# wongzbb/DiffMa-Diffusion-Mamba

Hardware: AMD Instinct MI355X
Metric: diffusion-steps/sec (DiffMa-L/2, 224x224, training; samples*steps/s) (higher is better)
Workload: dtype bf16 autocast (fp32 master weights, fp32 scan state); 1 GPU; DiffMa-L/2 DDP training step, 4x28x28 latents (196 tokens), batch 512/GPU; global_batch=512, seq_len=196, parallelism=dp1, gemm_tuning=file, world_size_seen_by_rccl=1

## Files before the change

### diffma-diffusion-mamba_amd/csrc/capi.hip

```cpp
#include "dm_common.h"
#include <cstdarg>
#include <cstdio>

namespace dm {
static thread_local char g_err[512] = "";
void set_error(const char* fmt, ...) {
    va_list ap;
    va_start(ap, fmt);
    vsnprintf(g_err, sizeof(g_err), fmt, ap);
    va_end(ap);
}
}

extern "C" int dm_abi_version(void) { return DM_ABI_VERSION; }
extern "C" const char* dm_last_error(void) { return dm::g_err; }
extern "C" const char* dm_build_info(void) {
#define DM_STR2(x) #x
#define DM_STR(x) DM_STR2(x)
    return "libdiffma_hip gfx950 (CDNA4, wave64) built " __DATE__ " " __TIME__ " hip " DM_STR(HIP_VERSION_MAJOR) "." DM_STR(
        HIP_VERSION_MINOR) "." DM_STR(HIP_VERSION_PATCH);
}
```

### diffma-diffusion-mamba_amd/csrc/conv_xproj.hip

```cpp
#include <cstdlib>
#include <type_traits>
#include "dm_mfma.h"

namespace dm {

constexpr int XP_TM = 16;
constexpr int XP_THREADS = 512;
constexpr int XP_PAD = 8;

template <typename T, typename TW, int W, bool SILU, int KSTEPS, bool IDX>
__global__ __launch_bounds__(XP_THREADS, 4) void conv_xproj_fwd_kernel(const dm_conv_xproj_fwd_args p) {
    constexpr int D = KSTEPS * 32;
    constexpr int KH = KSTEPS / 2;
    constexpr int ROW = D + XP_PAD;
    static_assert(KSTEPS % 2 == 0 && D <= 2 * XP_THREADS, "dim must be a multiple of 64 and at most 1024");
    __shared__ __attribute__((aligned(16))) uint16_t tile[2][XP_TM * ROW];
    __shared__ __attribute__((aligned(16))) f32x4 red[4][WAVE];

    const int tid = threadIdx.x;
    const int wave = __builtin_amdgcn_readfirstlane(tid >> 6), lane = tid & 63;
    const int nt = wave & 3, kh = wave >> 2;
    const int g = lane >> 4, ij = lane & 15;
    const int b = (int)blockIdx.x / p.ndir;
    const int dir = (int)blockIdx.x % p.ndir;
    const int s = dir * p.batch + b;
    const int L = p.seqlen;
    const cptr<int32_t> idx = IDX ? as_const(p.row_index + (int64_t)dir * L) : nullptr;
    const bool act = (D == 2 * XP_THREADS) ? true : (2 * tid < D);
    const int c = act ? 2 * tid : 0;
    const rsrc_t r_x = make_rsrc((const T*)p.x + (int64_t)b * p.x_sb);
    const rsrc_t r_o = make_rsrc((T*)p.out + (int64_t)s * p.o_ss);
    const int vo = c * (int)sizeof(T);
    const int sl_x = (int)p.x_sl * (int)sizeof(T), sl_o = (int)p.o_sl * (int)sizeof(T);
    const rsrc_t r_xd = make_rsrc((T*)p.xdbl + (int64_t)s * L * p.xd_sr);
    const int sr_xd = (int)p.xd_sr * (int)sizeof(T);

    const int ncol = p.nproj;
    const int col = nt * 16 + ij;
    const bool wave_on = nt * 16 < ncol;
    u32x4_t bfrag[KH];
    {
        const rsrc_t r_wx = __builtin_amdgcn_make_buffer_rsrc(const_cast<void*>(p.wx), 0, ncol * D * (int)sizeof(T), 0x00020000);
#pragma unroll
        for (int kk = 0; kk < KH; ++kk) {
            const auto q = __builtin_amdgcn_raw_buffer_load_b128(r_wx, (col * D + (kh * KH + kk) * 32 + g * 8) * (int)sizeof(T), 0, 0);
            bfrag[kk] = (u32x4_t){q[0], q[1], q[2], q[3]};
        }
    }

    float w[W][2], bias[2], win[W - 1][2];
#pragma unroll
    for (int v = 0; v < 2; ++v) {
#pragma unroll
        for (int j = 0; j < W; ++j) w[j][v] = io<TW>::ld((const TW*)p.weight + (int64_t)(c + v) * W + j);
        bias[v] = p.bias ? io<TW>::ld((const TW*)p.bias + c + v) : 0.0f;
#pragma unroll
        for (int j = 0; j < W - 1; ++j) win[j][v] = 0.0f;
    }

    auto load_half = [&](int l0, int h, uint32_t(&xin)[XP_TM]) {
#pragma unroll
        for (int j = h * (XP_TM / 2); j < (h + 1) * (XP_TM / 2); ++j) {
            int l = l0 + j;
            l = l < L ? l : L - 1;
            const int r = IDX ? idx[l] : l;
            xin[j] = __builtin_amdgcn_raw_buffer_load_b32(r_x, vo, r * sl_x, 0);
        }
    };
// ... 19 lines not shown
#pragma unroll
                for (int k = 0; k < W - 2; ++k) win[k][v] = win[k + 1][v];
                if (W > 1) win[W - 2][v] = xv[v];
            }
            const uint32_t pk = valid ? mfma<T>::pack(acc[0], acc[1]) : 0u;
            if (act) {
                *reinterpret_cast<uint32_t*>(tl + j * ROW + c) = pk;
                if (valid) __builtin_amdgcn_raw_buffer_store_b32(pk, r_o, vo, (l0 + j) * sl_o, 0);
            }
        }
        if (t + 1 < ntile) load_half(l0 + XP_TM, h, xin);
    };
    for (int t = 0; t < ntile; ++t) {
        const int l0 = t * XP_TM;
        uint16_t* const tl = tile[t & 1];
        conv_half(t, 0);
        conv_half(t, 1);
        __syncthreads();
        f32x4 acc = {0.f, 0.f, 0.f, 0.f};
        if (wave_on) {
#pragma unroll
            for (int kk = 0; kk < KH; ++kk) {
                const u32x4_t a = *reinterpret_cast<const u32x4_t*>(tl + ij * ROW + (kh * KH + kk) * 32 + g * 8);
                acc = mfma<T>::m16(a, bfrag[kk], acc);
            }
            if (kh == 1) red[nt][lane] = acc;
        }
        __syncthreads();
        if (wave_on && kh == 0 && col < ncol) {
            const f32x4 o = acc + red[nt][lane];
#pragma unroll
            for (int r = 0; r < 4; ++r) {
                const int l = l0 + 4 * g + r;
                if (l < L) bio<T>::st(r_xd, l * sr_xd + col * (int)sizeof(T), 0, o[r]);
            }
        }
    }
}

template <typename T, typename TW, int W, int KSTEPS>
static void launch_xp(const dm_conv_xproj_fwd_args& a, hipStream_t st) {
    dim3 grid(a.ndir * a.batch), block(XP_THREADS);
    const bool silu = (a.flags & DM_FLAG_SILU) != 0;
    if (a.row_index) {
        if (silu) hipLaunchKernelGGL((conv_xproj_fwd_kernel<T, TW, W, true, KSTEPS, true>), grid, block, 0, st, a);
        else hipLaunchKernelGGL((conv_xproj_fwd_kernel<T, TW, W, false, KSTEPS, true>), grid, block, 0, st, a);
    } else {
        if (silu) hipLaunchKernelGGL((conv_xproj_fwd_kernel<T, TW, W, true, KSTEPS, false>), grid, block, 0, st, a);
        else hipLaunchKernelGGL((conv_xproj_fwd_kernel<T, TW, W, false, KSTEPS, false>), grid, block, 0, st, a);
    }
}

template <typename T, typename TW, int W>
static int xp_by_dim(const dm_conv_xproj_fwd_args& a, hipStream_t st) {
    switch (a.dim) {
        case 1024: launch_xp<T, TW, W, 32>(a, st); break;
#ifndef DM_FAST_BUILD
        case 512: launch_xp<T, TW, W, 16>(a, st); break;
        case 256: launch_xp<T, TW, W, 8>(a, st); break;
#endif
        case 128: launch_xp<T, TW, W, 4>(a, st); break;
        default: set_error("dm_gather_conv1d_xproj_fwd: dim %d not instantiated (128, 256, 512, 1024)", a.dim); return DM_ERR_ARG;
    }
    return launch_status("dm_gather_conv1d_xproj_fwd");
}

template <typename T, typename TW>
// ... 8 lines not shown
    }
}

}

extern "C" int dm_gather_conv1d_xproj_width_supported(int width) {
#ifdef DM_FAST_BUILD
    return width == 4;
#else
    return width >= 2 && width <= 4;
#endif
}

extern "C" int dm_gather_conv1d_xproj_supported(int dim, int nproj, int io_dtype) {
    const bool d_ok = dim == 128 || dim == 256 || dim == 512 || dim == 1024;
    return (d_ok && nproj >= 1 && nproj <= 64 && (io_dtype == DM_BF16 || io_dtype == DM_F16)) ? 1 : 0;
}

extern "C" int dm_gather_conv1d_xproj_fwd(const dm_conv_xproj_fwd_args* args, void* stream) {
    using namespace dm;
    if (!args) { set_error("dm_gather_conv1d_xproj_fwd: null args"); return DM_ERR_ARG; }
    const dm_conv_xproj_fwd_args& a = *args;
    if (!a.x || !a.weight || !a.out || !a.wx || !a.xdbl) { set_error("dm_gather_conv1d_xproj_fwd: null tensor pointer"); return DM_ERR_ARG; }
    if (a.batch <= 0 || a.dim <= 0 || a.seqlen <= 0 || a.ndir <= 0) { set_error("dm_gather_conv1d_xproj_fwd: non-positive size"); return DM_ERR_ARG; }
    if (a.ndir > 1 && !a.row_index) { set_error("dm_gather_conv1d_xproj_fwd: ndir>1 needs row_index"); return DM_ERR_ARG; }
    if (!dm_gather_conv1d_xproj_supported(a.dim, a.nproj, a.io_dtype)) {
        set_error("dm_gather_conv1d_xproj_fwd: needs 16-bit I/O, dim in {128,256,512,1024}, nproj <= 64 (got dim %d nproj %d dtype %d)", a.dim, a.nproj, a.io_dtype);
        return DM_ERR_ARG;
    }
    if (a.x_sd != 1 || a.o_sd != 1) { set_error("dm_gather_conv1d_xproj_fwd: needs token-major tensors (channel stride 1)"); return DM_ERR_LAYOUT; }
    if (((uintptr_t)a.x & 3) || (a.x_sb & 1) || (a.x_sl & 1) || ((uintptr_t)a.out & 3) || (a.o_ss & 1) || (a.o_sl & 1) || ((uintptr_t)a.wx & 15)) {
        set_error("dm_gather_conv1d_xproj_fwd: x / out need 4-byte aligned rows, wx a 16-byte aligned base");
        return DM_ERR_LAYOUT;
    }
    hipStream_t st = (hipStream_t)stream;
    const bool wf32 = a.w_dtype == DM_F32;
    if (!wf32 && a.w_dtype != a.io_dtype) { set_error("dm_gather_conv1d_xproj_fwd: w_dtype must be fp32 or io_dtype"); return DM_ERR_DTYPE; }
    if (a.io_dtype == DM_BF16) return wf32 ? xp_by_width<bf16_t, float>(a, st) : xp_by_width<bf16_t, bf16_t>(a, st);
    return wf32 ? xp_by_width<f16_t, float>(a, st) : xp_by_width<f16_t, f16_t>(a, st);
}

namespace dm {

template <typename T, typename TW, int W, bool SILU, int D, bool IDX, bool MERGED = false>
__global__ __launch_bounds__(XP_THREADS, 2) void conv_xproj_bwd_kernel(const dm_conv_xproj_bwd_args p) {
    constexpr int NTW = D / 128;
    constexpr int ROWP = D + 4;
    constexpr int KP = 64;
    static_assert(D % 128 == 0 && D <= 2 * XP_THREADS, "dim must be a multiple of 128 and at most 1024");
    __shared__ __attribute__((aligned(16))) float ptile[XP_TM * ROWP];

    const int tid = threadIdx.x;
    const int wave = __builtin_amdgcn_readfirstlane(tid >> 6), lane = tid & 63;
    const int g = lane >> 4, ij = lane & 15;
    const int L = p.seqlen;
    const int b = MERGED ? (int)blockIdx.x : (int)blockIdx.x % p.batch;
    const bool act = (D == 2 * XP_THREADS) ? true : (2 * tid < D);
    const int c = act ? 2 * tid : 0;
    constexpr int ES = (int)sizeof(T);
    const rsrc_t r_x = make_rsrc((const T*)p.x + (int64_t)b * p.x_sb);
    const rsrc_t r_wt = make_rsrc(p.wxt);
    const int vo = c * ES;
    const int sl_x = (int)p.x_sl * ES, sl_du = (int)p.du_sl * ES, sl_dx = (int)p.dx_sl * ES, sr_xd = (int)p.xd_sr * ES;

    u32x4_t bfrag[NTW][2];
#pragma unroll
// ... 550 lines not shown
```

### diffma-diffusion-mamba_amd/csrc/dm_common.h

```cpp
#pragma once
#include <hip/hip_runtime.h>
#include <hip/hip_bf16.h>
#include <hip/hip_fp16.h>
#include <stdint.h>
#include "../../include/diffma_hip.h"

namespace dm {

constexpr int WAVE = 64;
constexpr float LOG2E = 1.4426950408889634f;
constexpr float LN2 = 0.6931471805599453f;

constexpr int DM_MAX_MIX = 2;
template <typename A> struct mix_args {
    A a[DM_MAX_MIX];
    int n;
};
void set_error(const char* fmt, ...);
static inline int launch_status(const char* who) {
    const hipError_t e = hipGetLastError();
    if (e == hipSuccess) return DM_OK;
    set_error("%s: launch failed: %s", who, hipGetErrorString(e));
    return DM_ERR_LAUNCH;
}
template <typename A> static inline mix_args<A> mix_make(const A& a, const A* second, unsigned& gz) {
    mix_args<A> m;
    m.a[0] = a;
    m.a[1] = second ? *second : a;
    m.n = second ? 2 : 1;
    gz = (unsigned)m.n;
    return m;
}
template <typename A, typename Check, typename Pairs, typename Run>
static inline int mix_run_n(const char* who, const A* args, int n, void* stream, Check check, Pairs pairs, Run run) {
    if (!args || n <= 0) { set_error("%s: null args / n <= 0", who); return DM_ERR_ARG; }
    for (int i = 0; i < n;) {
        int rc = check(args[i]);
        if (rc != 0) return rc;
        const bool pair = i + 1 < n && check(args[i + 1]) == 0 && pairs(args[i], args[i + 1]);
        rc = run(args[i], pair ? &args[i + 1] : nullptr, (hipStream_t)stream);
        if (rc != 0) return rc;
        i += pair ? 2 : 1;
    }
    return 0;
}
static inline bool same_align16(const void* x, const void* y) { return (((uintptr_t)x ^ (uintptr_t)y) & 15) == 0; }
static inline bool same_align4(const void* x, const void* y) { return (((uintptr_t)x ^ (uintptr_t)y) & 3) == 0; }
template <typename A, typename... M>
static inline bool mix_congruent(const A& x, const A& y, M A::*... ptrs) {
    if ((... || ((x.*ptrs == nullptr) != (y.*ptrs == nullptr)))) return false;
    A u = x, v = y;
    ((u.*ptrs = nullptr, v.*ptrs = nullptr), ...);
    return __builtin_memcmp(&u, &v, sizeof(A)) == 0;
}

typedef float f32x2 __attribute__((ext_vector_type(2)));
typedef float f32x4 __attribute__((ext_vector_type(4)));

struct bf16_t { uint16_t v; };
struct f16_t { _Float16 v; };

typedef __bf16 dm_bf16x2_t __attribute__((ext_vector_type(2)));
typedef float dm_f32x2_t __attribute__((ext_vector_type(2)));
__device__ __forceinline__ uint32_t dm_cvt_pk_bf16(float lo, float hi) {
    return __builtin_bit_cast(uint32_t, __builtin_convertvector((dm_f32x2_t){lo, hi}, dm_bf16x2_t));
}

__device__ __forceinline__ uint32_t f32_to_bf16_bits(float x) {
    return dm_cvt_pk_bf16(x, x) & 0xffffu;
}

template <typename T> struct io;
template <> struct io<float> {
    static __device__ __forceinline__ float ld(const float* p) { return *p; }
    static __device__ __forceinline__ void st(float* p, float x) { *p = x; }
    static __device__ __forceinline__ uint32_t ld_raw(const float* p) { return __float_as_uint(*p); }
    static __device__ __forceinline__ float cv(uint32_t w) { return __uint_as_float(w); }
};
template <> struct io<bf16_t> {
    static __device__ __forceinline__ float ld(const bf16_t* p) {
        return __uint_as_float(((uint32_t)p->v) << 16);
    }
    static __device__ __forceinline__ void st(bf16_t* p, float x) { p->v = (uint16_t)f32_to_bf16_bits(x); }
    static __device__ __forceinline__ uint32_t ld_raw(const bf16_t* p) { return (uint32_t)p->v; }
    static __device__ __forceinline__ float cv(uint32_t w) { return __uint_as_float(w << 16); }
};
template <> struct io<f16_t> {
    static __device__ __forceinline__ float ld(const f16_t* p) { return (float)p->v; }
    static __device__ __forceinline__ void st(f16_t* p, float x) { p->v = (_Float16)x; }
    static __device__ __forceinline__ uint32_t ld_raw(const f16_t* p) { return (uint32_t)__builtin_bit_cast(unsigned short, p->v); }
// ... 184 lines not shown
```

### diffma-diffusion-mamba_amd/csrc/scan_fwd_impl.h

```cpp
#pragma once
#include "dm_common.h"
#include <type_traits>

namespace dm {

#ifndef DM_FWD_F32_WAVES
#define DM_FWD_F32_WAVES 1
#endif

template <int N, bool HAS_Z, bool SOFTPLUS, bool ASH = false>
__device__ __forceinline__ float scan_step(f32x2 (&h)[N / 2], const f32x2 (&A2)[N / 2], const float (&Bv)[N],
                                           const float (&Cv)[N], float uu, float draw, float zz, float Dv, float bias) {
    float dl = draw + bias;
    if (SOFTPLUS) dl = softplus_f(dl);
    const float du = dl * uu;
    f32x2 acc = (f32x2){0.0f, 0.0f};
    float a_sh = 0.0f;
    if (ASH) a_sh = fast_exp2(A2[0].x * dl);
#pragma unroll
    for (int k = 0; k < N / 2; ++k) {
        f32x2 a;
        if (ASH) {
            a = (f32x2){a_sh, a_sh};
        } else {
            const f32x2 t = A2[k] * dl;
            a.x = fast_exp2(t.x);
            a.y = fast_exp2(t.y);
        }
        f32x2 bb, cc;
        bb.x = Bv[2 * k];
        bb.y = Bv[2 * k + 1];
        cc.x = Cv[2 * k];
        cc.y = Cv[2 * k + 1];
        h[k] = a * h[k] + bb * du;
        acc += h[k] * cc;
    }
    float y = acc.x + acc.y + Dv * uu;
    if (HAS_Z) y *= silu_f(zz);
    return y;
}

template <typename T, typename TBC, int N, bool HAS_Z, bool IDX, bool CKPT, bool SOFTPLUS, int PF, bool ASH = false, bool ACC = false>
__global__ __launch_bounds__(64) __attribute__((amdgpu_waves_per_eu((sizeof(T) == 2 && sizeof(TBC) == 2 && N <= 16) ? (ACC ? 3 : 4) : ((sizeof(T) == 4 && N <= 16) ? DM_FWD_F32_WAVES : 1)))) void scan_fwd_kernel(const dm_scan_fwd_args p) {
    static_assert(!ACC || IDX, "accumulating launches are built for the model's call pattern (row-index tables)");
    static_assert(N % 2 == 0, "d_state must be even");
    static_assert(PF == 8, "the B/C staging below maps 8 steps onto the 64 lanes");
    constexpr int NP = N / 2;
    constexpr int ES = (int)sizeof(T), EBC = (int)sizeof(TBC);
    constexpr int PER = N / 4;
    __shared__ __attribute__((aligned(16))) float bc_lds[2][PF][2 * N];
    const int d_raw = blockIdx.x * WAVE + threadIdx.x;
    const int d = (d_raw < p.dim) ? d_raw : p.dim - 1;
    const int L = p.seqlen;
    const int bpd = (p.batch_per_dir > 0) ? p.batch_per_dir : p.nseq;
    const int grp = (blockIdx.x * WAVE) / (p.dim / p.ngroups);
    const int s = blockIdx.y;
    const int dir = s / bpd;
    const int sb = s - dir * bpd;

    const rsrc_t r_u = make_rsrc((const T*)p.u + (int64_t)s * p.u_ss);
    const rsrc_t r_dt = make_rsrc((const T*)p.delta + (int64_t)s * p.dt_ss);
    const rsrc_t r_z = make_rsrc(HAS_Z ? (const T*)p.z + (int64_t)sb * p.z_ss : nullptr);
    const rsrc_t r_o = make_rsrc((T*)p.out + (int64_t)s * p.o_ss);
    const int vo = d * ES;
    const int sl_u = (int)p.u_sl * ES, sl_dt = (int)p.dt_sl * ES, sl_z = (int)p.z_sl * ES, sl_o = (int)p.o_sl * ES;
    const int lane = threadIdx.x;
    const int bc_step = lane >> 3, bc_part = lane & 7;
    const bool bc_isB = bc_part < 4;
    const rsrc_t r_bc = make_rsrc(bc_isB ? (const void*)((const TBC*)p.B + (int64_t)s * p.B_ss + (int64_t)grp * p.B_sg)
                                         : (const void*)((const TBC*)p.C + (int64_t)s * p.C_ss + (int64_t)grp * p.C_sg));
    const int sl_bc = (int)(bc_isB ? p.B_sl : p.C_sl) * EBC;
    const int vo_bc = (bc_part & 3) * PER * EBC;
    float* const bc_slot = &bc_lds[0][bc_step][(bc_isB ? 0 : N) + (bc_part & 3) * PER];
    const cptr<int32_t> zidx = IDX ? as_const(p.z_row_index + (int64_t)dir * L) : nullptr;
    const cptr<int32_t> oidx = IDX ? as_const(p.out_row_index + (int64_t)dir * L) : nullptr;

    f32x2 A2[NP];
#pragma unroll
    for (int j = 0; j < NP; ++j) {
        A2[j].x = p.A[(int64_t)d * N + 2 * j] * LOG2E;
        A2[j].y = p.A[(int64_t)d * N + 2 * j + 1] * LOG2E;
    }
    const float Dv = p.D ? p.D[d] : 0.0f;
    const float bias = p.delta_bias ? p.delta_bias[d] : 0.0f;

    f32x2 h[NP];
#pragma unroll
    for (int j = 0; j < NP; ++j) h[j] = (f32x2){0.0f, 0.0f};

    constexpr bool CK_PACKED = std::is_same<T, bf16_t>::value;
    constexpr int CK_ROWS = CK_PACKED ? NP : N;
    const int nchunk = CKPT ? (L + DM_SCAN_CKPT_EVERY - 1) / DM_SCAN_CKPT_EVERY : 0;
    const rsrc_t r_ck = make_rsrc(CKPT ? (const uint32_t*)p.ckpt + (int64_t)s * nchunk * CK_ROWS * p.dim : nullptr);
    auto store_slot = [&](int c) {
        if constexpr (CK_PACKED) {
            uint32_t w[NP];
#pragma unroll
            for (int k = 0; k < NP; ++k) asm("v_cvt_pk_bf16_f32 %0, %1, %2" : "=v"(w[k]) : "v"(h[k].x), "v"(h[k].y));
            bio_st_words<NP>(w, r_ck, d * 16, c * p.dim * NP * 4, p.dim * 16);
        } else {
#pragma unroll
            for (int k = 0; k < NP; ++k) {
                bio<float>::st(r_ck, d * 4, ((c * N + 2 * k) * p.dim) * 4, h[k].x);
                bio<float>::st(r_ck, d * 4, ((c * N + 2 * k + 1) * p.dim) * 4, h[k].y);
            }
        }
    };
    auto store_ckpt = [&](int done) {
        if (done < L) store_slot(done / DM_SCAN_CKPT_EVERY);
    };

    auto ld_old = [&](int l) -> float {
        if constexpr (ACC) return bio<T>::ld(r_o, vo, oidx[l] * sl_o);
        else return 0.0f;
    };
    float ru[PF], rd[PF], rz[PF], ro[ACC ? PF : 1];
#pragma unroll
    for (int j = 0; j < PF; ++j) {
        const int l = (j < L) ? j : L - 1;
        ru[j] = bio<T>::ld(r_u, vo, l * sl_u);
        rd[j] = bio<T>::ld(r_dt, vo, l * sl_dt);
        if (HAS_Z) rz[j] = bio<T>::ld(r_z, vo, (IDX ? zidx[l] : l) * sl_z);
        if (ACC) ro[j] = ld_old(l);
    }
    auto fetch_bc = [&](int l0, float(&v)[PER]) {
        int l = l0 + bc_step;
        l = (l < L) ? l : L - 1;
        bio_ld_vec<TBC, PER>(v, r_bc, vo_bc + l * sl_bc, 0);
    };
    auto stash_bc = [&](int b, const float(&v)[PER]) {
#pragma unroll
        for (int k = 0; k < PER; ++k) bc_slot[b * PF * 2 * N + k] = v[k];
    };
    {
        float v[PER];
        fetch_bc(0, v);
        stash_bc(0, v);
    }
    int buf = 0;

    auto run_block = [&](int l0, const float(&cu)[PF], const float(&cd)[PF], const float(&cz)[PF], const float(&co)[ACC ? PF : 1],
                         float(&nu)[PF], float(&nd)[PF], float(&nz)[PF], float(&no)[ACC ? PF : 1]) {
        float nbc[PER];
        fetch_bc(l0 + PF, nbc);
#pragma unroll
        for (int j = 0; j < PF; ++j) {
            int l = l0 + PF + j;
            l = (l < L) ? l : L - 1;
            nu[j] = bio<T>::ld(r_u, vo, l * sl_u);
            nd[j] = bio<T>::ld(r_dt, vo, l * sl_dt);
            if (HAS_Z) nz[j] = bio<T>::ld(r_z, vo, (IDX ? zidx[l] : l) * sl_z);
            if (ACC) no[j] = ld_old(l);
        }
#pragma unroll
        for (int j = 0; j < PF; ++j) {
            const int l = l0 + j;
            float Bc[N], Cc[N];
#pragma unroll
            for (int k = 0; k < N; ++k) {
                Bc[k] = bc_lds[buf][j][k];
                Cc[k] = bc_lds[buf][j][N + k];
            }
            float y = scan_step<N, HAS_Z, SOFTPLUS, ASH>(h, A2, Bc, Cc, cu[j], cd[j], HAS_Z ? cz[j] : 0.0f, Dv, bias);
            if (ACC) y += co[j];
            bio<T>::st(r_o, vo, (IDX ? oidx[l] : l) * sl_o, y);
            if (CKPT && (j + 1) % DM_SCAN_CKPT_EVERY == 0) store_ckpt(l0 + j + 1);
        }
        buf ^= 1;
        stash_bc(buf, nbc);
    };

    const int Lfull = (L / PF) * PF;
    float su[PF], sd[PF], sz[PF], so[ACC ? PF : 1];
    int l0 = 0;
    for (; l0 + 2 * PF <= Lfull; l0 += 2 * PF) {
        run_block(l0, ru, rd, rz, ro, su, sd, sz, so);
        run_block(l0 + PF, su, sd, sz, so, ru, rd, rz, ro);
    }
    if (l0 < Lfull) {
        run_block(l0, ru, rd, rz, ro, su, sd, sz, so);
#pragma unroll
        for (int j = 0; j < PF; ++j) {
            ru[j] = su[j];
            rd[j] = sd[j];
            if (HAS_Z) rz[j] = sz[j];
            if (ACC) ro[j] = so[j];
        }
    }
#pragma unroll
    for (int j = 0; j < PF; ++j) {
        const int l = Lfull + j;
        if (l < L) {
            float Bc[N], Cc[N];
#pragma unroll
            for (int k = 0; k < N; ++k) {
                Bc[k] = bc_lds[buf][j][k];
                Cc[k] = bc_lds[buf][j][N + k];
            }
            float y = scan_step<N, HAS_Z, SOFTPLUS, ASH>(h, A2, Bc, Cc, ru[j], rd[j], HAS_Z ? rz[j] : 0.0f, Dv, bias);
            if (ACC) y += ro[j];
            bio<T>::st(r_o, vo, (IDX ? oidx[l] : l) * sl_o, y);
            if (CKPT && (j + 1) % DM_SCAN_CKPT_EVERY == 0) store_ckpt(l + 1);
        }
    }

    if (CKPT) store_slot(0);

    if (p.last_state) {
        float* ls = p.last_state + ((int64_t)s * N) * p.dim + d;
#pragma unroll
        for (int k = 0; k < NP; ++k) {
            ls[(int64_t)(2 * k) * p.dim] = h[k].x;
            ls[(int64_t)(2 * k + 1) * p.dim] = h[k].y;
        }
    }
}

constexpr int SCAN_PF = 8;
static_assert(SCAN_PF % DM_SCAN_CKPT_EVERY == 0, "checkpoints fall on fixed positions of a prefetch block");

template <typename T, typename TBC, int N, bool HAS_Z, bool IDX>
static void launch_fwd3(const dm_scan_fwd_args& a, hipStream_t st, dim3 grid) {
    const bool sp = (a.flags & DM_FLAG_DELTA_SOFTPLUS) != 0;
    if constexpr (N == 16 && HAS_Z && IDX) {
        if ((a.flags & DM_FLAG_OUT_ACCUMULATE) && sp && !(a.flags & DM_FLAG_A_SHARED)) {
            if (a.ckpt) hipLaunchKernelGGL((scan_fwd_kernel<T, TBC, N, true, true, true, true, SCAN_PF, false, true>), grid, dim3(WAVE), 0, st, a);
            else hipLaunchKernelGGL((scan_fwd_kernel<T, TBC, N, true, true, false, true, SCAN_PF, false, true>), grid, dim3(WAVE), 0, st, a);
            return;
        }
    }
    if constexpr (N == 16 && HAS_Z && IDX) {
        if ((a.flags & DM_FLAG_A_SHARED) && sp) {
            if (a.ckpt) hipLaunchKernelGGL((scan_fwd_kernel<T, TBC, N, true, true, true, true, SCAN_PF, true>), grid, dim3(WAVE), 0, st, a);
            else hipLaunchKernelGGL((scan_fwd_kernel<T, TBC, N, true, true, false, true, SCAN_PF, true>), grid, dim3(WAVE), 0, st, a);
            return;
        }
    }
    if (a.ckpt) {
        if (sp) hipLaunchKernelGGL((scan_fwd_kernel<T, TBC, N, HAS_Z, IDX, true, true, SCAN_PF>), grid, dim3(WAVE), 0, st, a);
        else hipLaunchKernelGGL((scan_fwd_kernel<T, TBC, N, HAS_Z, IDX, true, false, SCAN_PF>), grid, dim3(WAVE), 0, st, a);
    } else {
        if (sp) hipLaunchKernelGGL((scan_fwd_kernel<T, TBC, N, HAS_Z, IDX, false, true, SCAN_PF>), grid, dim3(WAVE), 0, st, a);
        else hipLaunchKernelGGL((scan_fwd_kernel<T, TBC, N, HAS_Z, IDX, false, false, SCAN_PF>), grid, dim3(WAVE), 0, st, a);
    }
}

template <typename T, typename TBC, int N>
static int launch_fwd(const dm_scan_fwd_args& a, hipStream_t st) {
    dim3 grid((a.dim + WAVE - 1) / WAVE, a.nseq);
    const bool idx = a.z_row_index != nullptr;
    if (a.z) {
        if (idx) launch_fwd3<T, TBC, N, true, true>(a, st, grid);
        else launch_fwd3<T, TBC, N, true, false>(a, st, grid);
    } else {
        if (idx) launch_fwd3<T, TBC, N, false, true>(a, st, grid);
        else launch_fwd3<T, TBC, N, false, false>(a, st, grid);
    }
    return launch_status("dm_selective_scan_fwd");
}

template <typename T, typename TBC>
static int dispatch_n(const dm_scan_fwd_args& a, hipStream_t st) {
    switch (a.dstate) {
        case 16: return launch_fwd<T, TBC, 16>(a, st);
#ifndef DM_FAST_BUILD
        case 8: return launch_fwd<T, TBC, 8>(a, st);
        case 32: return launch_fwd<T, TBC, 32>(a, st);
        case 64: return launch_fwd<T, TBC, 64>(a, st);
#endif
        default:
            set_error("dm_selective_scan_fwd: d_state=%d not instantiated (8,16,32,64)", a.dstate);
            return DM_ERR_DSTATE;
    }
}

template <typename T>
static int dispatch_bc(const dm_scan_fwd_args& a, hipStream_t st) {
    if (a.bc_dtype == DM_F32) return dispatch_n<T, float>(a, st);
    if (a.bc_dtype == a.io_dtype) return dispatch_n<T, T>(a, st);
    set_error("dm_selective_scan_fwd: bc_dtype %d must be fp32 or equal io_dtype %d", a.bc_dtype, a.io_dtype);
    return DM_ERR_DTYPE;
}

// ... 2 lines not shown
```

### diffma-diffusion-mamba_amd/hip_ops.py

```python
from __future__ import annotations

import ctypes
import os
import threading

import torch

from . import _lib
from ._lib import (DM_BF16, DM_F16, DM_F32, DM_FLAG_A_SHARED, DM_FLAG_DELTA_ACTIVATED, DM_FLAG_DX_MERGED, DM_FLAG_PARTIAL_COMPACT, DM_FLAG_OUT_ACCUMULATE, DM_FLAG_DELTA_SOFTPLUS, DM_FLAG_DOUT_PER_SEQ, DM_FLAG_SCAN_CHUNKED, DM_FLAG_SCAN_SEQUENTIAL, DM_FLAG_SILU, dm_blend_args, dm_gate_head_args, dm_dtproj_bwd_args, dm_conv_bwd_args, dm_rmsnorm_merge_args, dm_colsum_args, dm_sum_partials_args,
                   dm_conv_fwd_args, dm_conv_xproj_bwd_args, dm_conv_xproj_fwd_args, dm_diffusion_step_args, dm_ln_mod_args, dm_ssd_bwd_args, dm_ssd_fwd_args, dm_merge_args, dm_gate_bwd_args, dm_dtproj_args, dm_scan_bwd_args, dm_scan_fwd_args, dm_gemm_args, dm_repack_args, dm_training_loss_args)

_DT = {torch.float32: DM_F32, torch.bfloat16: DM_BF16, torch.float16: DM_F16}
SCAN_CKPT_EVERY = _lib.DM_SCAN_CKPT_EVERY


def union_length(intervals):
    total, cur_s, cur_e = 0.0, None, None
    for s0, e0 in sorted(intervals):
        if cur_e is None or s0 > cur_e:
            if cur_e is not None:
                total += cur_e - cur_s
            cur_s, cur_e = s0, e0
        else:
            cur_e = max(cur_e, e0)
# ... 378 lines not shown
    Bsz, L, Dm = x.shape
    W = weight.shape[-1]
    weight = weight.reshape(Dm, W).contiguous()
    if weight.dtype != x.dtype and weight.dtype != torch.float32:
        weight = weight.float()
    if bias is not None:
        bias = bias.to(weight.dtype).contiguous()
    if out is None:
        out = torch.empty((ndir * Bsz, L, Dm), dtype=x.dtype, device=x.device)
    a = dm_conv_fwd_args()
    a.batch, a.dim, a.seqlen, a.width, a.ndir = Bsz, Dm, L, W, ndir
    a.io_dtype, a.w_dtype = dtype_code(x), dtype_code(weight)
    a.flags = DM_FLAG_SILU if silu else 0
    a.x, a.weight, a.bias, a.row_index, a.out = _ptr(x), _ptr(weight), _ptr(bias), _ptr(row_index), _ptr(out)
    a.x_sb, a.x_sl, a.x_sd = x.stride()
    a.o_ss, a.o_sl, a.o_sd = out.stride()
    _launch("dm_gather_conv1d_fwd", a, x, 2 * ndir * Bsz * L * Dm * x.element_size())
    return out


XPROJ_FUSED_MIN_SEQS = 512


def conv_xproj_supported(x, wx, nseq, width=4):
    if not x.is_cuda or x.dtype not in (torch.bfloat16, torch.float16) or nseq < XPROJ_FUSED_MIN_SEQS:
        return False
    if not _lib.load().dm_gather_conv1d_xproj_width_supported(int(width)):
        return False
    if x.stride(0) % 2 or x.stride(1) % 2 or x.storage_offset() % 2:
        return False
    return bool(_lib.load().dm_gather_conv1d_xproj_supported(int(x.shape[-1]), int(wx.shape[0]), dtype_code(x)))


def gather_conv1d_xproj_fwd(x, weight, bias, wx, *, row_index=None, ndir=1, silu=True):
    _require_gpu(x, weight, bias, wx)
    Bsz, L, Dm = x.shape
    W = weight.shape[-1]
    P = wx.shape[0]
    weight = weight.reshape(Dm, W).contiguous()
    if weight.dtype != x.dtype and weight.dtype != torch.float32:
        weight = weight.float()
    if bias is not None:
        bias = bias.to(weight.dtype).contiguous()
    wx = wx.contiguous()
    assert wx.dtype == x.dtype and wx.shape[1] == Dm
    out = torch.empty((ndir * Bsz, L, Dm), dtype=x.dtype, device=x.device)
    xdbl = torch.empty((ndir * Bsz * L, P), dtype=x.dtype, device=x.device)
    a = dm_conv_xproj_fwd_args()
    a.batch, a.dim, a.seqlen, a.width, a.ndir = Bsz, Dm, L, W, ndir
    a.io_dtype, a.w_dtype = dtype_code(x), dtype_code(weight)
    a.flags = DM_FLAG_SILU if silu else 0
    a.nproj = P
    a.x, a.weight, a.bias, a.row_index = _ptr(x), _ptr(weight), _ptr(bias), _ptr(row_index)
    a.wx, a.out, a.xdbl = _ptr(wx), _ptr(out), _ptr(xdbl)
    a.x_sb, a.x_sl, a.x_sd = x.stride()
    a.o_ss, a.o_sl, a.o_sd = out.stride()
    a.xd_sr = P
    es = x.element_size()
    _launch("dm_gather_conv1d_xproj_fwd", a, x, 2 * ndir * Bsz * L * Dm * es + ndir * Bsz * L * P * es + P * Dm * es)
    return out, xdbl


XPROJ_FUSED_BWD = os.environ.get("DIFFMA_FUSED_CONV_BWD", "1") == "1"


def conv_xproj_bwd_supported(x, wx, nseq, width=4, du=None, dxdbl=None):
    if not XPROJ_FUSED_BWD:
        return False
    if not _lib.load().dm_gather_conv1d_xproj_width_supported(int(width)):
        return False
    if du is not None and (du.data_ptr() % 4 or du.stride(0) % 2 or du.stride(1) % 2 or du.stride(2) != 1):
        return False
    if dxdbl is not None and (dxdbl.data_ptr() % 16 or dxdbl.stride(0) % 8 or dxdbl.stride(1) != 1):
        return False
    if not x.is_cuda or x.dtype not in (torch.bfloat16, torch.float16) or nseq < XPROJ_FUSED_MIN_SEQS:
        return False
    if x.stride(0) % 2 or x.stride(1) % 2 or x.storage_offset() % 2:
        return False
    return bool(_lib.load().dm_gather_conv1d_xproj_bwd_supported(int(x.shape[-1]), int(wx.shape[0]), dtype_code(x)))


DX_MERGED = os.environ.get("DIFFMA_DX_MERGED", "1") == "1"


def gather_conv1d_xproj_bwd(x, weight, bias, du, dxdbl, wxt, *, row_index=None, ndir=1, silu=True, merged_out=None):
    _require_gpu(x, weight, bias, du, dxdbl, wxt)
    Bsz, L, Dm = x.shape
    W = weight.shape[-1]
    P = wxt.shape[1]
    weight = weight.reshape(Dm, W).contiguous()
    if weight.dtype != x.dtype and weight.dtype != torch.float32:
        weight = weight.float()
    if bias is not None:
# ... 632 lines not shown
```

### diffma-diffusion-mamba_amd/selective_scan_interface.py

```python
from __future__ import annotations

import os

import torch
import torch.nn.functional as F

from . import _lib, hip_ops
from .step_prep import cast_weight, stacked_pair


REPACK_OWN = os.environ.get("DIFFMA_REPACK_OWN", "1") == "1"


def _repack_own(t: torch.Tensor) -> bool:
    return (REPACK_OWN and t.is_cuda and t.dim() == 3 and t.stride(2) == 1 and t.shape[0] <= 65535
            and t.dtype in (torch.float32, torch.bfloat16, torch.float16))


def _to_token_major(t: torch.Tensor) -> torch.Tensor:
    tm = t.transpose(1, 2)
    if tm.stride(-1) == 1:
        return tm
    if _repack_own(t):
        return hip_ops.repack(t, True)
# ... 232 lines not shown
                    dx = GemmChain.run(F.linear, dy2c, wt).view(xc.shape).to(x_dt)
            else:
                dx = GemmChain.run(torch.mm, dy2, wc).view(xc.shape).to(x_dt)
            if not ctx.needs_input_grad[1]:
                dw = None
            elif b_dt is None and _own_single(dy2c, x2c, False, False, torch.float32):
                dw = hip_ops.gemm(dy2c, x2c, False, False, out_dtype=torch.float32).to(w_dt)
            else:
                dw = _tn_splitk(dy2c, x2c).to(w_dt)
            db = dy2.sum(0, dtype=torch.float32).to(b_dt) if (b_dt is not None and ctx.needs_input_grad[2]) else None
        return dx, dw, db


def linear_splitk(x, weight, bias=None):
    return _LinearSplitKFn.apply(x, weight, bias)


HOIST_GATE = os.environ.get("DIFFMA_HOIST_GATE", "1") == "1"


class _SpiralSSMFn(torch.autograd.Function):

    @staticmethod
    def forward(ctx, xz, conv_w, conv_b, Wx, Wdt, dt_bias, A, Dskip, scan_index, grad_on=True, out_index=None, merge=True):
        Bsz, L, D2 = xz.shape
        Din = D2 // 2
        ndir = scan_index.shape[0]
        R = Wdt.shape[1]
        N = A.shape[1]
        dt_ = xz.dtype
        x_view, z_view = xz[..., :Din], xz[..., Din:]
        need_grad = grad_on and (ctx.needs_input_grad[0] or any(ctx.needs_input_grad[1:8]))
        Wx_c, Wdt_c = cast_weight(Wx, dt_), cast_weight(Wdt, dt_)
        if hip_ops.conv_xproj_supported(x_view, Wx_c, ndir * Bsz, conv_w.shape[-1]):
            xc, x_dbl = hip_ops.gather_conv1d_xproj_fwd(x_view, conv_w, conv_b, Wx_c, row_index=scan_index, ndir=ndir, silu=True)
        else:
            xc = hip_ops.gather_conv1d_fwd(x_view, conv_w, conv_b, row_index=scan_index, ndir=ndir, silu=True)
            x_dbl = GemmChain.run(F.linear, xc.view(-1, Din), Wx_c)
        hoist = HOIST_GATE and merge and out_index is None and (ndir > 1 or Bsz >= hip_ops.XPROJ_FUSED_MIN_SEQS)
        act = hoist and N == 16 and hip_ops.dtproj_softplus_supported(x_dbl, Wdt_c)
        if act:
            delta = hip_ops.dtproj_softplus_fwd(x_dbl, Wdt_c, dt_bias).view(ndir * Bsz, L, Din)
        else:
            delta = GemmChain.run(F.linear, x_dbl[:, :R], Wdt_c).view(ndir * Bsz, L, Din)
        xd3 = x_dbl.view(ndir * Bsz, L, R + 2 * N)
        Bm, Cm = xd3[..., R:R + N], xd3[..., R + N:]
        ckpt = None
        if need_grad:
            ckpt = hip_ops.alloc_scan_ckpt(ndir * Bsz, L, N, Din, xz.dtype, xz.device)
        oidx = scan_index if out_index is None else out_index
        ctx.merge, ctx.hoist, ctx.act = merge, hoist, act
        if hoist:
            ydir = hip_ops.scan_fwd(xc, delta, A, Bm, Cm, Dskip, None, dt_bias, True, z_row_index=scan_index, out_row_index=oidx,
                                    batch_per_dir=Bsz, ckpt=ckpt, delta_activated=act)
            pre = torch.empty((Bsz, L, Din), dtype=dt_, device=xz.device) if need_grad else None
            y = hip_ops.token_merge(ydir.view(ndir, Bsz, L, Din), gate=z_view, pre_out=pre)
            ctx.save_for_backward(xz, conv_w, conv_b, Wx, Wdt, dt_bias, A, Dskip, scan_index, xc, x_dbl, delta, ckpt, Wx_c, Wdt_c, oidx, pre)
            return y
        ydir = hip_ops.scan_fwd(xc, delta, A, Bm, Cm, Dskip, z_view, dt_bias, True, z_row_index=scan_index,
                                out_row_index=oidx, batch_per_dir=Bsz, ckpt=ckpt)
        ctx.save_for_backward(xz, conv_w, conv_b, Wx, Wdt, dt_bias, A, Dskip, scan_index, xc, x_dbl, delta, ckpt, Wx_c, Wdt_c, oidx, None)
        if not merge:
            return ydir.view(ndir, Bsz, L, Din)
        return hip_ops.token_merge(ydir.view(ndir, Bsz, L, Din)) if ndir > 1 else ydir

    @staticmethod
    def backward(ctx, dy):
        xz, conv_w, conv_b, Wx, Wdt, dt_bias, A, Dskip, scan_index, xc, x_dbl, delta, ckpt, Wx_c, Wdt_c, oidx, pre = ctx.saved_tensors
        Bsz, L, D2 = xz.shape
        Din = D2 // 2
        ndir = scan_index.shape[0]
        R = Wdt.shape[1]
        N = A.shape[1]
        dt_ = xz.dtype
        dy = dy.contiguous()
        if dy.dtype != dt_:
            dy = dy.to(dt_)
        if not ctx.merge:
            dy = dy.view(ndir * Bsz, L, Din)
# ... 507 lines not shown
```

### include/diffma_hip.h

```cpp
#ifndef DIFFMA_HIP_H
#define DIFFMA_HIP_H

#include <stdint.h>

#ifdef __cplusplus
extern "C" {
#endif

#define DM_ABI_VERSION 29

typedef enum {
    DM_OK = 0,
    DM_ERR_ARG = -1,
    DM_ERR_LAYOUT = -2,
    DM_ERR_DTYPE = -3,
    DM_ERR_DSTATE = -4,
    DM_ERR_LAUNCH = -5
} dm_status;

typedef enum { DM_F32 = 0, DM_BF16 = 1, DM_F16 = 2 } dm_dtype;

enum {
    DM_FLAG_DELTA_SOFTPLUS = 1,
    DM_FLAG_SILU = 2,
    DM_FLAG_A_SHARED = 8,
    DM_FLAG_DOUT_PER_SEQ = 4,
    DM_FLAG_SCAN_SEQUENTIAL = 16,
    DM_FLAG_SCAN_CHUNKED = 32,
    DM_FLAG_OUT_ACCUMULATE = 64,
    DM_FLAG_DX_MERGED = 256,
    DM_FLAG_PARTIAL_COMPACT = 512,
    DM_FLAG_DELTA_ACTIVATED = 128
};

typedef struct {
    int32_t batch, channels, hw, T;
    int32_t out_dtype, _pad;
    int32_t row_sqrt_ac, row_sqrt_1mac, row_post_logvar, row_log_betas, row_sqrt_recip_ac, row_sqrt_recipm1_ac, row_coef1, row_coef2;
    const void *model_out;
    const float *x_start, *x_t, *noise;
    const int64_t *t;
    const float *tables;
// ... 103 lines not shown
    const void *weight;
    const void *bias;
    const int32_t *row_index;
    void *out;
    int64_t x_sb, x_sl, x_sd;
    int64_t o_ss, o_sl, o_sd;
} dm_conv_fwd_args;

int dm_gather_conv1d_fwd(const dm_conv_fwd_args *args, void *stream);

typedef struct {
    int32_t batch, dim, seqlen, width, ndir;
    int32_t io_dtype, w_dtype;
    int32_t flags;
    int32_t nchunk;
    const void *x, *weight, *bias, *dout;
    const int32_t *row_index;
    void *dx;
    float *dw_partial, *db_partial;
    int64_t x_sb, x_sl, x_sd;
    int64_t do_ss, do_sl, do_sd;
    int64_t dx_ss, dx_sl, dx_sd;
    int64_t part_ss;
} dm_conv_bwd_args;

int dm_gather_conv1d_bwd(const dm_conv_bwd_args *args, void *stream);
int dm_conv_nchunk(int seqlen);

typedef struct {
    int32_t batch, dim, seqlen, width, ndir;
    int32_t io_dtype, w_dtype;
    int32_t flags;
    int32_t nproj;
    int32_t _pad;
    const void *x;
    const void *weight;
    const void *bias;
    const int32_t *row_index;
    const void *wx;
    void *out;
    void *xdbl;
    int64_t x_sb, x_sl, x_sd;
    int64_t o_ss, o_sl, o_sd;
    int64_t xd_sr;
} dm_conv_xproj_fwd_args;

int dm_gather_conv1d_xproj_fwd(const dm_conv_xproj_fwd_args *args, void *stream);
int dm_gather_conv1d_xproj_supported(int dim, int nproj, int io_dtype);
int dm_gather_conv1d_xproj_width_supported(int width);

typedef struct {
    int32_t batch, dim, seqlen, width, ndir;
    int32_t io_dtype, w_dtype;
    int32_t flags;
    int32_t nproj;
    int32_t _pad;
    const void *x, *weight, *bias;
    const int32_t *row_index;
    const void *du;
    const void *dxdbl;
    const void *wxt;
    void *dx;
    float *dw_partial, *db_partial;
    int64_t x_sb, x_sl, x_sd;
    int64_t du_ss, du_sl, du_sd;
    int64_t dx_ss, dx_sl, dx_sd;
    int64_t xd_sr;
    int64_t part_ss;
} dm_conv_xproj_bwd_args;

int dm_gather_conv1d_xproj_bwd(const dm_conv_xproj_bwd_args *args, void *stream);
int dm_gather_conv1d_xproj_bwd_supported(int dim, int nproj, int io_dtype);
int dm_gather_conv1d_xproj_bwd_slab(const dm_conv_xproj_bwd_args *args, void *stream);

typedef struct {
    int32_t nin, batch, seqlen, dim;
    int32_t io_dtype, out_dtype;
// ... 252 lines not shown
```

Baseline: 2492 samples*steps/s.

## Emit fp32 B/C rows from conv-xproj and read them via scalar loads in scan

Measured after the change: 2488 samples*steps/s. No clear change (-0.2%).

```diff
diff --git a/diffma-diffusion-mamba_amd/csrc/capi.hip b/diffma-diffusion-mamba_amd/csrc/capi.hip
--- a/diffma-diffusion-mamba_amd/csrc/capi.hip
+++ b/diffma-diffusion-mamba_amd/csrc/capi.hip
@@ -1,6 +1,7 @@
 #include "dm_common.h"
 #include <cstdarg>
 #include <cstdio>
+#include <cstdlib>
 
 namespace dm {
 static thread_local char g_err[512] = "";
@@ -9,6 +10,10 @@
     va_start(ap, fmt);
     vsnprintf(g_err, sizeof(g_err), fmt, ap);
     va_end(ap);
+}
+int scan_bc_scalar_mask() {
+    const char* e = getenv("DIFFMA_SCAN_BC_SCALAR");
+    return e ? atoi(e) : 1;
 }
 }
 
diff --git a/diffma-diffusion-mamba_amd/csrc/conv_xproj.hip b/diffma-diffusion-mamba_amd/csrc/conv_xproj.hip
--- a/diffma-diffusion-mamba_amd/csrc/conv_xproj.hip
+++ b/diffma-diffusion-mamba_amd/csrc/conv_xproj.hip
@@ -34,6 +34,10 @@
     const int sl_x = (int)p.x_sl * (int)sizeof(T), sl_o = (int)p.o_sl * (int)sizeof(T);
     const rsrc_t r_xd = make_rsrc((T*)p.xdbl + (int64_t)s * L * p.xd_sr);
     const int sr_xd = (int)p.xd_sr * (int)sizeof(T);
+    const bool bc_on = p.bc_f32 != nullptr;
+    const rsrc_t r_bc = __builtin_amdgcn_make_buffer_rsrc(p.bc_f32 ? p.bc_f32 + (int64_t)s * L * p.bc_sr : nullptr, 0,
+                                                          bc_on ? (int)(L * p.bc_sr * 4) : 0, 0x00020000);
+    const int sr_bc = (int)p.bc_sr * 4;
 
     const int ncol = p.nproj;
     const int col = nt * 16 + ij;
@@ -119,7 +123,14 @@
 #pragma unroll
             for (int r = 0; r < 4; ++r) {
                 const int l = l0 + 4 * g + r;
-                if (l < L) bio<T>::st(r_xd, l * sr_xd + col * (int)sizeof(T), 0, o[r]);
+                if (l < L) {
+                    bio<T>::st(r_xd, l * sr_xd + col * (int)sizeof(T), 0, o[r]);
+                    if (bc_on && col >= p.bc_col0) {
+                        T rounded;
+                        io<T>::st(&rounded, o[r]);
+                        __builtin_amdgcn_raw_buffer_store_b32(__float_as_uint(io<T>::ld(&rounded)), r_bc, l * sr_bc + (col - p.bc_col0) * 4, 0, 0);
+                    }
+                }
             }
         }
     }
@@ -194,6 +205,11 @@
     if (((uintptr_t)a.x & 3) || (a.x_sb & 1) || (a.x_sl & 1) || ((uintptr_t)a.out & 3) || (a.o_ss & 1) || (a.o_sl & 1) || ((uintptr_t)a.wx & 15)) {
         set_error("dm_gather_conv1d_xproj_fwd: x / out need 4-byte aligned rows, wx a 16-byte aligned base");
         return DM_ERR_LAYOUT;
+    }
+    if (a.bc_f32 && (a.bc_col0 < 0 || a.bc_col0 >= a.nproj || a.bc_sr < a.nproj - a.bc_col0 || ((uintptr_t)a.bc_f32 & 3) ||
+                     (int64_t)a.seqlen * a.bc_sr * 4 > 0x7fffffffLL)) {
+        set_error("dm_gather_conv1d_xproj_fwd: bc_f32 needs 0 <= bc_col0 < nproj, bc_sr >= nproj - bc_col0, a 4-byte aligned base, seqlen * bc_sr * 4 < 2^31");
+        return DM_ERR_ARG;
     }
     hipStream_t st = (hipStream_t)stream;
     const bool wf32 = a.w_dtype == DM_F32;
diff --git a/diffma-diffusion-mamba_amd/csrc/dm_common.h b/diffma-diffusion-mamba_amd/csrc/dm_common.h
--- a/diffma-diffusion-mamba_amd/csrc/dm_common.h
+++ b/diffma-diffusion-mamba_amd/csrc/dm_common.h
@@ -44,6 +44,11 @@
     }
     return 0;
 }
+int scan_bc_scalar_mask();
+static inline bool scan_bc_scalar_ok(int bc_dtype, int dstate, int ngroups, int flags, const void* B, const void* C, int64_t B_sn, int64_t C_sn) {
+    return bc_dtype == DM_F32 && dstate == 16 && ngroups == 1 && !(flags & (DM_FLAG_A_SHARED | DM_FLAG_OUT_ACCUMULATE)) && B_sn == 1 && C_sn == 1 &&
+           (((uintptr_t)B | (uintptr_t)C) & 3) == 0;
+}
 static inline bool same_align16(const void* x, const void* y) { return (((uintptr_t)x ^ (uintptr_t)y) & 15) == 0; }
 static inline bool same_align4(const void* x, const void* y) { return (((uintptr_t)x ^ (uintptr_t)y) & 3) == 0; }
 template <typename A, typename... M>
@@ -56,6 +61,10 @@
 
 typedef float f32x2 __attribute__((ext_vector_type(2)));
 typedef float f32x4 __attribute__((ext_vector_type(4)));
+typedef float f32x8 __attribute__((ext_vector_type(8)));
+typedef float f32x16 __attribute__((ext_vector_type(16)));
+typedef f32x8 f32x8_a4 __attribute__((aligned(4)));
+typedef f32x16 f32x16_a4 __attribute__((aligned(4)));
 
 struct bf16_t { uint16_t v; };
 struct f16_t { _Float16 v; };
diff --git a/diffma-diffusion-mamba_amd/csrc/scan_fwd_impl.h b/diffma-diffusion-mamba_amd/csrc/scan_fwd_impl.h
--- a/diffma-diffusion-mamba_amd/csrc/scan_fwd_impl.h
+++ b/diffma-diffusion-mamba_amd/csrc/scan_fwd_impl.h
@@ -40,15 +40,16 @@
     return y;
 }
 
-template <typename T, typename TBC, int N, bool HAS_Z, bool IDX, bool CKPT, bool SOFTPLUS, int PF, bool ASH = false, bool ACC = false>
-__global__ __launch_bounds__(64) __attribute__((amdgpu_waves_per_eu((sizeof(T) == 2 && sizeof(TBC) == 2 && N <= 16) ? (ACC ? 3 : 4) : ((sizeof(T) == 4 && N <= 16) ? DM_FWD_F32_WAVES : 1)))) void scan_fwd_kernel(const dm_scan_fwd_args p) {
+template <typename T, typename TBC, int N, bool HAS_Z, bool IDX, bool CKPT, bool SOFTPLUS, int PF, bool ASH = false, bool ACC = false, bool SBC = false>
+__global__ __launch_bounds__(64) __attribute__((amdgpu_waves_per_eu((sizeof(T) == 2 && (sizeof(TBC) == 2 || SBC) && N <= 16) ? (ACC ? 3 : 4) : ((sizeof(T) == 4 && N <= 16) ? DM_FWD_F32_WAVES : 1)))) void scan_fwd_kernel(const dm_scan_fwd_args p) {
     static_assert(!ACC || IDX, "accumulating launches are built for the model's call pattern (row-index tables)");
+    static_assert(!SBC || (std::is_same<TBC, float>::value && N == 16 && !ASH && !ACC), "the scalar route is built for fp32 rows of 16 states");
     static_assert(N % 2 == 0, "d_state must be even");
     static_assert(PF == 8, "the B/C staging below maps 8 steps onto the 64 lanes");
     constexpr int NP = N / 2;
     constexpr int ES = (int)sizeof(T), EBC = (int)sizeof(TBC);
     constexpr int PER = N / 4;
-    __shared__ __attribute__((aligned(16))) float bc_lds[2][PF][2 * N];
+    __shared__ __attribute__((aligned(16))) float bc_lds[SBC ? 1 : 2][SBC ? 1 : PF][SBC ? 1 : 2 * N];
     const int d_raw = blockIdx.x * WAVE + threadIdx.x;
     const int d = (d_raw < p.dim) ? d_raw : p.dim - 1;
     const int L = p.seqlen;
@@ -74,6 +75,17 @@
     float* const bc_slot = &bc_lds[0][bc_step][(bc_isB ? 0 : N) + (bc_part & 3) * PER];
     const cptr<int32_t> zidx = IDX ? as_const(p.z_row_index + (int64_t)dir * L) : nullptr;
     const cptr<int32_t> oidx = IDX ? as_const(p.out_row_index + (int64_t)dir * L) : nullptr;
+    const cptr<float> Bsc = as_const((const float*)p.B + (int64_t)s * p.B_ss + (int64_t)grp * p.B_sg);
+    const cptr<float> Csc = as_const((const float*)p.C + (int64_t)s * p.C_ss + (int64_t)grp * p.C_sg);
+    const uint32_t sl_Bs = (uint32_t)p.B_sl * 4u;
+    constexpr int SBC_NU = 2, SBC_W = N / SBC_NU;
+    typedef float sbc_vec __attribute__((ext_vector_type(SBC_W)));
+    typedef sbc_vec sbc_vec_a4 __attribute__((aligned(4)));
+    auto ld_bc_piece = [&](int l, int u, sbc_vec& b, sbc_vec& c) {
+        const uint32_t off = (uint32_t)((l < L) ? l : L - 1) * sl_Bs + 4u * SBC_W * u;
+        b = *(const volatile sbc_vec_a4 __attribute__((address_space(4)))*)((cptr<char>)Bsc + off);
+        c = *(const volatile sbc_vec_a4 __attribute__((address_space(4)))*)((cptr<char>)Csc + off);
+    };
 
     f32x2 A2[NP];
 #pragma unroll
@@ -132,42 +144,100 @@
 #pragma unroll
         for (int k = 0; k < PER; ++k) bc_slot[b * PF * 2 * N + k] = v[k];
     };
-    {
+    sbc_vec Bq[SBC_NU + 1], Cq[SBC_NU + 1];
+    int orow = 0, orow_nx = 0;
+#pragma unroll
+    for (int u = 0; u <= SBC_NU; ++u) { Bq[u] = sbc_vec{}; Cq[u] = sbc_vec{}; }
+    if constexpr (SBC) {
+#pragma unroll
+        for (int u = 0; u < SBC_NU; ++u) ld_bc_piece(0, u, Bq[u], Cq[u]);
+        if (IDX) orow_nx = oidx[0];
+    } else {
         float v[PER];
         fetch_bc(0, v);
         stash_bc(0, v);
     }
     int buf = 0;
-
+    constexpr int SBC_FENCE = 0x7CF;
+    auto sbc_step = [&](int l, float uu, float draw, float zz) -> float {
+        float dl = draw + bias;
+        if (SOFTPLUS) dl = softplus_f(dl);
+        const float du = dl * uu;
+        f32x2 acc = (f32x2){0.0f, 0.0f};
+#pragma unroll
+        for (int u = 0; u < SBC_NU; ++u) {
+            __builtin_amdgcn_sched_barrier(SBC_FENCE);
+            ld_bc_piece(l + 1, u, Bq[SBC_NU], Cq[SBC_NU]);
+            if (IDX && u == 0) {
+                orow = orow_nx;
+                orow_nx = *(const volatile int32_t __attribute__((address_space(4)))*)(oidx + (uint32_t)((l + 1 < L) ? l + 1 : L - 1));
+            }
+            __builtin_amdgcn_sched_barrier(SBC_FENCE);
+#pragma unroll
+            for (int kk = 0; kk < SBC_W / 2; ++kk) {
+                const int k = (SBC_W / 2) * u + kk;
+                const f32x2 t = A2[k] * dl;
+                f32x2 a, bb, cc;
+                a.x = fast_exp2(t.x);
+                a.y = fast_exp2(t.y);
+                bb.x = Bq[0][2 * kk];
+                bb.y = Bq[0][2 * kk + 1];
+                cc.x = Cq[0][2 * kk];
+                cc.y = Cq[0][2 * kk + 1];
+                h[k] = a * h[k] + bb * du;
+                acc += h[k] * cc;
+            }
+#pragma unroll
+            for (int v = 0; v < SBC_NU; ++v) { Bq[v] = Bq[v + 1]; Cq[v] = Cq[v + 1]; }
+        }
+        float y = acc.x + acc.y + Dv * uu;
+        if (HAS_Z) y *= silu_f(zz);
+        return y;
+    };
+    auto step = [&](int l, int j, float uu, float draw, float zz) -> float {
+        if constexpr (SBC) {
+            if (!IDX) orow = l;
+            return sbc_step(l, uu, draw, zz);
+        } else {
+            orow = IDX ? oidx[l] : l;
+            float Bc[N], Cc[N];
+#pragma unroll
+            for (int k = 0; k < N; ++k) {
+                Bc[k] = bc_lds[buf][j][k];
+                Cc[k] = bc_lds[buf][j][N + k];
+            }
+            return scan_step<N, HAS_Z, SOFTPLUS, ASH>(h, A2, Bc, Cc, uu, draw, zz, Dv, bias);
+        }
+    };
     auto run_block = [&](int l0, const float(&cu)[PF], const float(&cd)[PF], const float(&cz)[PF], const float(&co)[ACC ? PF : 1],
                          float(&nu)[PF], float(&nd)[PF], float(&nz)[PF], float(&no)[ACC ? PF : 1]) {
         float nbc[PER];
-        fetch_bc(l0 + PF, nbc);
-#pragma unroll
-        for (int j = 0; j < PF; ++j) {
+        if constexpr (!SBC) fetch_bc(l0 + PF, nbc);
+        auto request = [&](int j) {
             int l = l0 + PF + j;
             l = (l < L) ? l : L - 1;
             nu[j] = bio<T>::ld(r_u, vo, l * sl_u);
             nd[j] = bio<T>::ld(r_dt, vo, l * sl_dt);
             if (HAS_Z) nz[j] = bio<T>::ld(r_z, vo, (IDX ? zidx[l] : l) * sl_z);
             if (ACC) no[j] = ld_old(l);
+        };
+        if constexpr (!SBC) {
+#pragma unroll
+            for (int j = 0; j < PF; ++j) request(j);
         }
 #pragma unroll
         for (int j = 0; j < PF; ++j) {
             const int l = l0 + j;
-            float Bc[N], Cc[N];
-#pragma unroll
-            for (int k = 0; k < N; ++k) {
-                Bc[k] = bc_lds[buf][j][k];
-                Cc[k] = bc_lds[buf][j][N + k];
-            }
-            float y = scan_step<N, HAS_Z, SOFTPLUS, ASH>(h, A2, Bc, Cc, cu[j], cd[j], HAS_Z ? cz[j] : 0.0f, Dv, bias);
+            float y = step(l, j, cu[j], cd[j], HAS_Z ? cz[j] : 0.0f);
             if (ACC) y += co[j];
-            bio<T>::st(r_o, vo, (IDX ? oidx[l] : l) * sl_o, y);
+            bio<T>::st(r_o, vo, orow * sl_o, y);
             if (CKPT && (j + 1) % DM_SCAN_CKPT_EVERY == 0) store_ckpt(l0 + j + 1);
-        }
-        buf ^= 1;
-        stash_bc(buf, nbc);
+            if constexpr (SBC) request(j);
+        }
+        if constexpr (!SBC) {
+            buf ^= 1;
+            stash_bc(buf, nbc);
+        }
     };
 
     const int Lfull = (L / PF) * PF;
@@ -191,23 +261,18 @@
     for (int j = 0; j < PF; ++j) {
         const int l = Lfull + j;
         if (l < L) {
-            float Bc[N], Cc[N];
-#pragma unroll
-            for (int k = 0; k < N; ++k) {
-                Bc[k] = bc_lds[buf][j][k];
-                Cc[k] = bc_lds[buf][j][N + k];
-            }
-            float y = scan_step<N, HAS_Z, SOFTPLUS, ASH>(h, A2, Bc, Cc, ru[j], rd[j], HAS_Z ? rz[j] : 0.0f, Dv, bias);
+            float y = step(l, j, ru[j], rd[j], HAS_Z ? rz[j] : 0.0f);
             if (ACC) y += ro[j];
-            bio<T>::st(r_o, vo, (IDX ? oidx[l] : l) * sl_o, y);
+            bio<T>::st(r_o, vo, orow * sl_o, y);
             if (CKPT && (j + 1) % DM_SCAN_CKPT_EVERY == 0) store_ckpt(l + 1);
         }
     }
 
     if (CKPT) store_slot(0);
 
-    if (p.last_state) {
-        float* ls = p.last_state + ((int64_t)s * N) * p.dim + d;
+    float* const last_state = SBC ? nullptr : p.last_state;
+    if (last_state) {
+        float* ls = last_state + ((int64_t)s * N) * p.dim + d;
 #pragma unroll
         for (int k = 0; k < NP; ++k) {
             ls[(int64_t)(2 * k) * p.dim] = h[k].x;
@@ -245,10 +310,38 @@
     }
 }
 
+template <typename T, bool HAS_Z, bool IDX, bool CKPT, bool SP>
+constexpr bool sbc_fwd_built() {
+    if (HAS_Z || !CKPT) return false;
+    if (std::is_same<T, bf16_t>::value) return IDX && !SP;
+    if (std::is_same<T, float>::value) return IDX || !SP;
+    return false;
+}
+template <typename T, bool IDX, bool SP>
+static bool launch_fwd_sbc2(const dm_scan_fwd_args& a, hipStream_t st, dim3 grid) {
+    if constexpr (sbc_fwd_built<T, false, IDX, true, SP>()) {
+        hipLaunchKernelGGL((scan_fwd_kernel<T, float, 16, false, IDX, true, SP, SCAN_PF, false, false, true>), grid, dim3(WAVE), 0, st, a);
+        return true;
+    }
+    return false;
+}
+template <typename T>
+static bool launch_fwd_sbc(const dm_scan_fwd_args& a, hipStream_t st, dim3 grid) {
+    if (a.z || !a.ckpt) return false;
+    const bool sp = (a.flags & DM_FLAG_DELTA_SOFTPLUS) != 0;
+    if (a.z_row_index) return sp ? launch_fwd_sbc2<T, true, true>(a, st, grid) : launch_fwd_sbc2<T, true, false>(a, st, grid);
+    return sp ? launch_fwd_sbc2<T, false, true>(a, st, grid) : launch_fwd_sbc2<T, false, false>(a, st, grid);
+}
+
 template <typename T, typename TBC, int N>
 static int launch_fwd(const dm_scan_fwd_args& a, hipStream_t st) {
     dim3 grid((a.dim + WAVE - 1) / WAVE, a.nseq);
     const bool idx = a.z_row_index != nullptr;
+    if constexpr (std::is_same<TBC, float>::value && N == 16) {
+        if ((scan_bc_scalar_mask() & 1) && !a.last_state && a.B_sl == a.C_sl && a.B_sl >= 0 && (int64_t)a.seqlen * a.B_sl * 4 < 0x7fffffffLL &&
+            scan_bc_scalar_ok(a.bc_dtype, a.dstate, a.ngroups, a.flags, a.B, a.C, a.B_sn, a.C_sn) && launch_fwd_sbc<T>(a, st, grid))
+            return launch_status("dm_selective_scan_fwd");
+    }
     if (a.z) {
         if (idx) launch_fwd3<T, TBC, N, true, true>(a, st, grid);
         else launch_fwd3<T, TBC, N, true, false>(a, st, grid);
diff --git a/diffma-diffusion-mamba_amd/hip_ops.py b/diffma-diffusion-mamba_amd/hip_ops.py
--- a/diffma-diffusion-mamba_amd/hip_ops.py
+++ b/diffma-diffusion-mamba_amd/hip_ops.py
@@ -434,7 +434,10 @@
     return bool(_lib.load().dm_gather_conv1d_xproj_supported(int(x.shape[-1]), int(wx.shape[0]), dtype_code(x)))
 
 
-def gather_conv1d_xproj_fwd(x, weight, bias, wx, *, row_index=None, ndir=1, silu=True):
+SCAN_BC_SCALAR = int(os.environ.get("DIFFMA_SCAN_BC_SCALAR", "1"))
+
+
+def gather_conv1d_xproj_fwd(x, weight, bias, wx, *, row_index=None, ndir=1, silu=True, bc_rows_from=None):
     _require_gpu(x, weight, bias, wx)
     Bsz, L, Dm = x.shape
     W = weight.shape[-1]
@@ -459,8 +462,14 @@
     a.o_ss, a.o_sl, a.o_sd = out.stride()
     a.xd_sr = P
     es = x.element_size()
-    _launch("dm_gather_conv1d_xproj_fwd", a, x, 2 * ndir * Bsz * L * Dm * es + ndir * Bsz * L * P * es + P * Dm * es)
-    return out, xdbl
+    nbytes = 2 * ndir * Bsz * L * Dm * es + ndir * Bsz * L * P * es + P * Dm * es
+    bc = None
+    if bc_rows_from is not None:
+        assert 0 <= bc_rows_from < P
+        bc = torch.empty((ndir * Bsz * L, P - bc_rows_from), dtype=torch.float32, device=x.device)
+        a.bc_f32, a.bc_col0, a.bc_sr = _ptr(bc), bc_rows_from, P - bc_rows_from
+    _launch("dm_gather_conv1d_xproj_fwd", a, x, nbytes, None if bc is None else nbytes + bc.numel() * 4)
+    return (out, xdbl) if bc is None else (out, xdbl, bc)
 
 
 XPROJ_FUSED_BWD = os.environ.get("DIFFMA_FUSED_CONV_BWD", "1") == "1"
diff --git a/diffma-diffusion-mamba_amd/selective_scan_interface.py b/diffma-diffusion-mamba_amd/selective_scan_interface.py
--- a/diffma-diffusion-mamba_amd/selective_scan_interface.py
+++ b/diffma-diffusion-mamba_amd/selective_scan_interface.py
@@ -288,8 +288,13 @@
         x_view, z_view = xz[..., :Din], xz[..., Din:]
         need_grad = grad_on and (ctx.needs_input_grad[0] or any(ctx.needs_input_grad[1:8]))
         Wx_c, Wdt_c = cast_weight(Wx, dt_), cast_weight(Wdt, dt_)
+        bc32 = None
         if hip_ops.conv_xproj_supported(x_view, Wx_c, ndir * Bsz, conv_w.shape[-1]):
-            xc, x_dbl = hip_ops.gather_conv1d_xproj_fwd(x_view, conv_w, conv_b, Wx_c, row_index=scan_index, ndir=ndir, silu=True)
+            if hip_ops.SCAN_BC_SCALAR & 1 and N == 16:
+                xc, x_dbl, bc32 = hip_ops.gather_conv1d_xproj_fwd(x_view, conv_w, conv_b, Wx_c, row_index=scan_index, ndir=ndir, silu=True,
+                                                                  bc_rows_from=R)
+            else:
+                xc, x_dbl = hip_ops.gather_conv1d_xproj_fwd(x_view, conv_w, conv_b, Wx_c, row_index=scan_index, ndir=ndir, silu=True)
         else:
             xc = hip_ops.gather_conv1d_fwd(x_view, conv_w, conv_b, row_index=scan_index, ndir=ndir, silu=True)
             x_dbl = GemmChain.run(F.linear, xc.view(-1, Din), Wx_c)
@@ -301,6 +306,9 @@
             delta = GemmChain.run(F.linear, x_dbl[:, :R], Wdt_c).view(ndir * Bsz, L, Din)
         xd3 = x_dbl.view(ndir * Bsz, L, R + 2 * N)
         Bm, Cm = xd3[..., R:R + N], xd3[..., R + N:]
+        if bc32 is not None:
+            bc3 = bc32.view(ndir * Bsz, L, 2 * N)
+            Bm, Cm = bc3[..., :N], bc3[..., N:]
         ckpt = None
         if need_grad:
             ckpt = hip_ops.alloc_scan_ckpt(ndir * Bsz, L, N, Din, xz.dtype, xz.device)
diff --git a/include/diffma_hip.h b/include/diffma_hip.h
--- a/include/diffma_hip.h
+++ b/include/diffma_hip.h
@@ -7,7 +7,7 @@
 extern "C" {
 #endif
 
-#define DM_ABI_VERSION 29
+#define DM_ABI_VERSION 30
 
 typedef enum {
     DM_OK = 0,
@@ -177,7 +177,7 @@
     int32_t io_dtype, w_dtype;
     int32_t flags;
     int32_t nproj;
-    int32_t _pad;
+    int32_t bc_col0;
     const void *x;
     const void *weight;
     const void *bias;
@@ -188,6 +188,8 @@
     int64_t x_sb, x_sl, x_sd;
     int64_t o_ss, o_sl, o_sd;
     int64_t xd_sr;
+    float *bc_f32;
+    int64_t bc_sr;
 } dm_conv_xproj_fwd_args;
 
 int dm_gather_conv1d_xproj_fwd(const dm_conv_xproj_fwd_args *args, void *stream);
```
